# bupt-ai-cz/HIAST

Measured on AMD Instinct MI355X. Metric: self-training images/sec (fwd+bwd+pseudo-label) at 1024x512, higher is better.
Workload: dtype fp16

## Files before the change

hiast_amd/_lib.py:

```python
import ctypes
import os

import torch

_HERE = os.path.dirname(os.path.abspath(__file__))
LIB_PATH = os.environ.get("HIAST_LIB") or os.path.join(_HERE, "csrc", "libhiast_hip.so")

c_int, c_i64, c_f32, c_sz, c_vp = (ctypes.c_int, ctypes.c_int64, ctypes.c_float, ctypes.c_size_t,
                                   ctypes.c_void_p)

SIGNATURES = {
    "hiast_version": (c_int, []),
    "hiast_error_string": (ctypes.c_char_p, [c_int]),
    "hiast_upsample_bilinear_ac_fwd": (c_int, [c_vp, c_vp] + [c_int] * 6 + [c_vp]),
    "hiast_upsample_bilinear_ac_bwd": (c_int, [c_vp, c_vp] + [c_int] * 6 + [c_vp]),
    "hiast_plabel_pass1_workspace_bytes": (c_sz, [c_int]),
    "hiast_plabel_pass1": (c_int, [c_vp] + [c_int] * 6 + [c_vp, c_vp, c_vp, c_vp, c_sz, c_vp]),
    "hiast_plabel_pass2": (c_int, [c_vp, c_vp, c_vp, c_int, c_int, c_i64, c_vp, c_vp, c_vp, c_vp]),
    "hiast_plabel_strided_hist_workspace_bytes": (c_sz, [c_i64, c_int]),
    "hiast_plabel_strided_hist": (c_int, [c_vp, c_vp, c_i64, c_int, c_int, c_vp, c_vp, c_vp, c_vp, c_sz, c_vp]),
    "hiast_tta_fused": (c_int, [c_vp] * 6 + [c_int] * 5 + [c_vp, c_vp, c_vp]),
    "hiast_dinput_fwd": (c_int, [c_vp, c_int, c_vp] + [c_int] * 6 + [c_vp]),
    "hiast_dinput_bwd": (c_int, [c_vp, c_int, c_vp, c_vp, c_vp] + [c_int] * 6 + [c_vp]),
    "hiast_st_loss_workspace_bytes": (c_sz, [c_int] * 6),
# ... 39 lines not shown
    "hiast_conv_wgrad_nhwc": (c_int, [c_vp, c_vp, c_vp] + [c_int] * 9 + [c_vp, c_sz, c_vp]),
    "hiast_conv_wgrad_group_workspace_bytes": (c_sz, [c_vp, c_int]),
    "hiast_conv_wgrad_group_nhwc": (c_int, [c_vp, c_int, c_int, c_vp, c_sz, c_vp]),
    "hiast_conv_wgrad_small_workspace_bytes": (c_sz, [c_int] * 6),
    "hiast_conv_wgrad_small_nhwc": (c_int, [c_vp, c_vp, c_vp] + [c_int] * 9 + [c_vp, c_sz, c_vp]),
    "hiast_pack_conv_weight": (c_int, [c_vp, c_int, c_int, c_int, c_int, c_int, c_vp, c_vp, c_vp]),
    "hiast_bn_nhwc_workspace_bytes": (c_sz, [c_int]),
    "hiast_bn_nhwc_stats": (c_int, [c_vp, c_i64, c_int, c_vp, c_vp, c_sz, c_int, c_vp]),
    "hiast_bn_nhwc_apply": (c_int, [c_vp] * 8 + [ctypes.c_double, c_f32, c_f32, c_int, c_vp, c_vp, c_i64, c_int, c_vp,
                                    c_int, c_vp]),
    "hiast_bn_nhwc_apply_partial": (c_int, [c_vp] * 8 + [c_int, ctypes.c_double, c_f32, c_f32, c_int, c_vp, c_vp, c_i64,
                                            c_int, c_vp, c_int, c_vp]),
    "hiast_bn_nhwc_bwd_stats": (c_int, [c_vp] * 7 + [c_int, c_i64, c_int, c_vp, c_vp, c_sz, c_int, c_vp]),
    "hiast_bn_nhwc_bwd_apply": (c_int, [c_vp] * 8 + [ctypes.c_double, c_int, c_vp, c_vp, c_vp, c_vp, c_i64, c_int, c_int,
                                        c_vp]),
    "hiast_pack_conv_weight_multi": (c_int, [c_vp, c_vp, c_vp, c_int, c_int, c_vp]),
    "hiast_split_planes": (c_int, [c_vp, c_vp, c_i64, c_int, c_int, c_vp]),
    "hiast_stem_tail": (c_int, [c_vp, c_int, c_vp, c_vp, c_vp, c_vp, c_f32, c_vp, c_int, c_int, c_int, c_int, c_int, c_vp]),
    "hiast_stem_eval": (c_int, [c_vp] * 6 + [c_f32, c_vp, c_int, c_int, c_int, c_int, c_vp]),
    "hiast_stem_train_blocks": (c_int, [c_int] * 3),
    "hiast_stem_train_fwd": (c_int, [c_vp, c_vp, c_vp, c_vp, c_int, c_int, c_int, c_int, c_vp]),
    "hiast_stem_wgrad_workspace_bytes": (c_sz, [c_int] * 3),
    "hiast_stem_wgrad": (c_int, [c_vp, c_vp, c_vp, c_int, c_int, c_int, c_int, c_vp, c_sz, c_vp]),
    "hiast_ema_update": (c_int, [c_vp, c_vp, c_vp, c_int, c_f32, c_f32, c_vp]),
    "hiast_normalize_u8": (c_int, [c_vp, c_vp, c_int, c_i64, c_vp, c_vp, c_vp]),
    "hiast_maxpool3x3s2_nhwc_fwd": (c_int, [c_vp, c_vp, c_vp, c_int, c_int, c_int, c_int, c_int, c_vp]),
    "hiast_maxpool3x3s2_nhwc_bwd": (c_int, [c_vp, c_vp, c_vp, c_int, c_int, c_int, c_int, c_int, c_vp]),
    "hiast_multi_copy": (c_int, [c_vp, c_int, c_vp]),
    "hiast_aug_geometry_u8": (c_int, [c_vp] * 6 + [c_int] * 4 + [c_vp]),
    "hiast_aug_hist_u8": (c_int, [c_vp] * 5 + [c_int, c_i64, c_vp]),
# ... 70 lines not shown
```

hiast_amd/csrc/bn_nhwc.hip:

```cpp
#include <hip/hip_bf16.h>

#include "common.h"

namespace hiast {

constexpr int BNH_MAXBLK = 512;
#ifndef BNH_ROWS_PER_BLOCK_PASS
#define BNH_ROWS_PER_BLOCK_PASS 16
#endif
#ifndef BNH_APPLY_MAXBLK
#define BNH_APPLY_MAXBLK 65535
#endif
#ifndef BNH_CONTIG
#define BNH_CONTIG 0
#endif
#if BNH_CONTIG
#define BNH_ROW_WALK(CHUNK)                                                                                              \
    const long long step = (CHUNK);                                                                                      \
    const long long per_blk = ((M + gridDim.x - 1) / gridDim.x + (CHUNK) - 1) / (CHUNK) * (CHUNK);                       \
    const long long lim = (long long)(blockIdx.x + 1) * per_blk < M ? (long long)(blockIdx.x + 1) * per_blk : M;         \
    long long r0 = (long long)blockIdx.x * per_blk + rsub;
#else
#define BNH_ROW_WALK(CHUNK)                                                                                              \
    const long long step = (long long)gridDim.x * (CHUNK);                                                               \
// ... 382 lines not shown
            for (int k = 0; k < 8; ++k) {
                const bool open = GATE == 0 || (GATE == 1 ? yy[k] > 0.f
                                                : (GATE == 3 ? ((bits >> k) & 1u) != 0u : fmaf(xx[k], k0[k], gsh[k]) > 0.f));
                const float gg = open ? g[k] : 0.f;
                g[k] = gg;
                xx[k] = k0[k] * (gg - mg[k] - (xx[k] - mean[k]) * invstd[k] * mgx[k]);
            }
            bnh_store8<F16>(dx + off, xx, nt_out);
            if (DRES) bnh_store8<F16>(dres + off, g, nt_out);
        }
        r0 += step;
        if (r0 < lim) load_rows(r0);
    }
}

static int bnh_nblk(long long M, int C)
{
    const int rpp = 256 / (C / 8);
    long long nb = (M + (long long)rpp * 16 - 1) / ((long long)rpp * 16);
    nb = nb < 1 ? 1 : (nb > BNH_MAXBLK ? BNH_MAXBLK : nb);
    return (int)nb;
}

}

static bool bnh_c_ok(int C) { return C >= 8 && C <= 2048 && (C & (C - 1)) == 0; }

static int bnh_check(const void* x, long long M, int C)
{
    if (!x) return HIAST_E_ARG;
// ... 153 lines not shown
#define L1(G, DRES, F)                                                                                             \
    hipLaunchKernelGGL((hiast::bnh_bwd_apply_kernel<G, DRES, F>), dim3((unsigned)nb), dim3(256), 0, st,             \
                       (const unsigned short*)dy, (const unsigned short*)y, (const unsigned short*)x, gamma, beta,  \
                       save_mean, save_invstd, sums, 1.0 / count, (unsigned short*)dx, (unsigned short*)dres, dgamma, \
                       dbeta, (long long)M, C)
#define L(G, DRES) do { if (f16) L1(G, DRES, true); else L1(G, DRES, false); } while (0)
    if (relu == 1) { if (dres) L(1, true); else L(1, false); }
    else if (relu == 3) { if (dres) L(3, true); else L(3, false); }
    else if (relu == 2) { if (dres) L(2, true); else L(2, false); }
    else { if (dres) L(0, true); else L(0, false); }
#undef L
#undef L1
    HIAST_CHECK_LAUNCH();
    return 0;
}
```

hiast_amd/csrc/misc.hip:

```cpp
#include <hip/hip_bf16.h>

#include <atomic>

#include "common.h"

namespace hiast {

__global__ __launch_bounds__(256) void ema_kernel(const hiast_ema_rec* __restrict__ table,
                                                  const int32_t* __restrict__ chunk_tensor,
                                                  const int64_t* __restrict__ chunk_start,
                                                  float gamma, float omg)
{
    const hiast_ema_rec r = table[chunk_tensor[blockIdx.x]];
    const int64_t s = chunk_start[blockIdx.x];
    const int64_t e = (s + 65536 < r.n) ? s + 65536 : r.n;
    float* __restrict__ d = r.ema;
    const float* __restrict__ p = r.p;
    const bool vec = ((((uintptr_t)d) | ((uintptr_t)p)) & 15) == 0;
    if (vec) {
        const int64_t nv = (e - s) / 4;
        float4* d4 = reinterpret_cast<float4*>(d + s);
        const float4* p4 = reinterpret_cast<const float4*>(p + s);
        for (int64_t i = threadIdx.x; i < nv; i += 256) {
            float4 a = d4[i], b = p4[i];
// ... 348 lines not shown
                for (int k = 0; k < 8; ++k) {
                    const unsigned code = ((k < 4 ? cd.x : cd.y) >> (8 * (k & 3))) & 255u;
                    const float gv = (k & 1) ? H16<F16>::hi(gw[k >> 1]) : H16<F16>::lo(gw[k >> 1]);
                    if (code == pos) acc[k] += gv;
                }
            }
        }
        unsigned pk[4];
#pragma unroll
        for (int q = 0; q < 4; ++q)
            pk[q] = H16<F16>::pack(acc[2 * q], acc[2 * q + 1]);
        *reinterpret_cast<uint4*>(dx + (size_t)pix * C + cg * 8) = make_uint4(pk[0], pk[1], pk[2], pk[3]);
    }
}

}

static int maxpool_cl_check(const void* a, const void* b, const void* c, int B, int H, int W, int C)
{
    if (!a || !b || !c) return HIAST_E_ARG;
    if (B <= 0 || H <= 0 || W <= 0 || C <= 0) return HIAST_E_ARG;
    if (C % 8 != 0 || ((((uintptr_t)a) | ((uintptr_t)b)) & 15) || (((uintptr_t)c) & 7) ||
        (long long)B * H * W * C >= (1ll << 40))
        return HIAST_E_RANGE;
    return 0;
}

extern "C" int hiast_maxpool3x3s2_nhwc_fwd(const void* x, void* y, uint8_t* idx, int B, int H, int W, int C, int fmt,
                                           hiast_stream_t stream)
{
// ... 33 lines not shown
}

extern "C" int hiast_normalize_u8(const uint8_t* img, float* out, int B, int64_t HW, const float* mean, const float* std,
                                  hiast_stream_t stream)
{
    if (!img || !out || !mean || !std) return HIAST_E_ARG;
    if (B <= 0 || HW <= 0) return HIAST_E_ARG;
    if (B > 65535) return HIAST_E_RANGE;
    long long nb = (HW + 256 * 4 - 1) / (256 * 4);
    nb = nb < 1 ? 1 : (nb > 1024 ? 1024 : nb);
    hipLaunchKernelGGL(hiast::normalize_u8_kernel, dim3((unsigned)nb, B), dim3(256), 0, (hipStream_t)stream, img, out,
                       (long long)HW, mean[0], mean[1], mean[2], std[0], std[1], std[2]);
    HIAST_CHECK_LAUNCH();
    return 0;
}
```

hiast_amd/functional.py:

```python
import os

import torch

from . import kernels as K
from . import switches as SW

ASPP_DILATIONS = (6, 12, 18, 24)
H16 = (torch.bfloat16, torch.float16)


class _AsppFn(torch.autograd.Function):

    @staticmethod
    @torch.amp.custom_fwd(device_type="cuda", cast_inputs=torch.float32)
    def forward(ctx, x, w0, w1, w2, w3, b0, b1, b2, b3, dil):
        x = x.contiguous()
        ws = [w.contiguous() for w in (w0, w1, w2, w3)]
        bs = [b.contiguous() for b in (b0, b1, b2, b3)]
        wpack = K.aspp_pack_weights(ws, bs)
        Cout = ws[0].shape[0]
        y = K.aspp_fwd(x, wpack, Cout, dil)
        ctx.save_for_backward(x, wpack)
        ctx.dil = dil
        ctx.cin = x.shape[1]
# ... 299 lines not shown
        else:
            if fused is not None:
                sums = K.bn_nhwc_stats_from_partial(fused)
            else:
                sums = K.bn_nhwc_bwd_stats(dy, y, x, gamma, beta, sm, si, ctx.gate)
            if ctx.world != 1:
                _stat_all_reduce(sums)
        want_p = gamma is not None and (ctx.needs_input_grad[2] or ctx.needs_input_grad[3])
        handoff = ctx.box is not None and ctx.needs_input_grad[1]
        dx, dres, dg, db = K.bn_nhwc_bwd_apply(dy, y, x, gamma, beta, sm, si, sums, ctx.count, ctx.gate,
                                               ctx.has_res and ctx.needs_input_grad[1] and not handoff, want_p)
        if handoff:
            ctx.box["gated"] = (dy, y)
        return (dx, dres, dg if ctx.needs_input_grad[2] else None, db if ctx.needs_input_grad[3] else None,
                None, None, None, None, None, None, None, None, None)


class _ConvNhwcFn(torch.autograd.Function):

    @staticmethod
    @torch.amp.custom_fwd(device_type="cuda")
    def forward(ctx, x, weight, stride, dil, want_stats, box, packed, in_bn=None, wgroup=None, xsum=None, in_bn3=None):
        xv = x.permute(0, 2, 3, 1)
        ctx.in_bn3 = None
        if (in_bn3 is not None and "bn3" in in_bn3 and box is not None and stride == 1 and weight.shape[2] == 1
                and ctx.needs_input_grad[0] and _BN3_FUSION
                and K.xconv_dgrad_gated_bn_stats_ok(x.shape[0] * x.shape[2] * x.shape[3], weight.shape[0], weight.shape[1])):
            ctx.in_bn3 = in_bn3
        ctx.wgroup = wgroup
        ctx.xsum = xsum if (xsum is not None and stride == 1 and ctx.needs_input_grad[0]) else None
# ... 412 lines not shown
            dy = dy.to(ctx.dtype)
        return K.maxpool3x3s2_cl_bwd(dy.contiguous(memory_format=torch.channels_last), idx, *ctx.hw)


def maxpool(x, pool):
    if (x.is_cuda and x.dtype in H16 and _is_cl(x) and x.shape[1] % 8 == 0
            and (pool.kernel_size, pool.stride, pool.padding, pool.dilation, pool.ceil_mode) == (3, 2, 1, 1, False)
            and not pool.return_indices and os.environ.get("HIAST_LIB_MAXPOOL", "0") != "1"):
        return _MaxPool3x3s2ClFn.apply(x)
    return pool(x)


class _SubsampleClFn(torch.autograd.Function):

    @staticmethod
    def forward(ctx, x, s):
        ctx.s, ctx.shape = s, x.shape
        return x[:, :, ::s, ::s].contiguous(memory_format=torch.channels_last)

    @staticmethod
    def backward(ctx, dy):
        g = torch.empty(ctx.shape, dtype=dy.dtype, device=dy.device, memory_format=torch.channels_last).zero_()
        g[:, :, ::ctx.s, ::ctx.s] = dy
        return g, None


def conv_nhwc(x, conv, want_stats=False, box=None, in_bn=None, wgroup=None, xsum=None, in_bn3=None):
    w = conv.weight
    wv = w if wgroup is None else wgroup[2]
    fmt = K.fmt_of(x)
    fwd = conv.__dict__.get("_hiast_packed", {}).get(fmt)
    adj = conv.__dict__.get("_hiast_packed_adj", {}).get(fmt)
    ok = lambda e: e is not None and e[0] == w._version and e[1] == w.data_ptr()
    packed = (fwd[2] if ok(fwd) else None, adj[2] if ok(adj) else None)
    stride = conv.stride[0]
    if conv.kernel_size == (1, 1) and stride != 1:
        x = _SubsampleClFn.apply(x, stride)
        stride = 1
    return _ConvNhwcFn.apply(x, wv, stride, conv.dilation[0], bool(want_stats), box, packed, in_bn,
                             None if wgroup is None else (wgroup[0], wgroup[1]), xsum, in_bn3)


_nbt_batched = [False]


def bn_act(x, bn, res=None, relu=True, partial=None, box=None, stat_box=None):
    training = bn.training or (bn.running_mean is None)
    if training and bn.track_running_stats and bn.num_batches_tracked is not None and not _nbt_batched[0]:
        bn.num_batches_tracked.add_(1)
    momentum = 0.1 if bn.momentum is None else bn.momentum
    if (training and x.dtype in H16 and _is_cl(x) and not x.is_contiguous()
            and K.bn_nhwc_supported(x.shape[1]) and (res is None or (res.dtype == x.dtype and _is_cl(res)))):
        return _BnActNhwcFn.apply(x, res, bn.weight, bn.bias, bn.running_mean, bn.running_var, momentum, bn.eps, relu,
# ... 4 lines not shown
```

hiast_amd/kernels.py:

```python
import ctypes

import numpy as np
import torch

from . import _lib
from . import switches as _SW
from ._lib import NBINS, check


def _stream():
    return ctypes.c_void_p(torch._C._cuda_getCurrentRawStream(torch._C._cuda_getDevice()))


def _ptr(t):
    return ctypes.c_void_p(t.data_ptr()) if t is not None else ctypes.c_void_p(0)


def h2d_async(host, device, out=None):
    stage = torch.from_numpy(np.ascontiguousarray(host)).pin_memory()
    if out is None:
        return stage.to(device, non_blocking=True)
    out.copy_(stage.view(out.dtype).reshape(out.shape) if stage.dtype != out.dtype else stage.reshape(out.shape),
              non_blocking=True)
    return out
# ... 1310 lines not shown
def bn_nhwc_bwd_apply(dy, y, x, gamma, beta, save_mean, save_invstd, sums, count, gate, want_dres, want_dparam):
    xv, M, C = _bnh_view(x, "x")
    dv = _bnh_view(dy, "dy")[0]
    yv = _bnh_view(y, "y")[0] if gate == 1 else (_req(y, torch.uint8, 2, "mask") if gate == 3 else None)
    dx = torch.empty_like(x, memory_format=torch.channels_last)
    dres = torch.empty_like(x, memory_format=torch.channels_last) if want_dres else None
    dg = torch.empty(C, dtype=torch.float32, device=x.device) if want_dparam else None
    db = torch.empty(C, dtype=torch.float32, device=x.device) if want_dparam else None
    check(_lib.load().hiast_bn_nhwc_bwd_apply(_ptr(dv), _ptr(yv), _ptr(xv), _ptr(gamma), _ptr(beta), _ptr(save_mean),
                                              _ptr(save_invstd), _ptr(sums), float(count), int(gate), _ptr(dx),
                                              _ptr(dres), _ptr(dg), _ptr(db), M, C, fmt_of(x), _stream()),
          "hiast_bn_nhwc_bwd_apply")
    return dx, dres, dg, db


_wgrad_ws = {}


def conv_wgrad_supported(Cin, Cout, k, stride):
    return Cin % 256 == 0 and Cout % 256 == 0 and k in (1, 3) and (k == 3 or stride == 1)


def conv_wgrad_preferred(Cin, Cout, k, stride):
    import os
    if not conv_wgrad_supported(Cin, Cout, k, stride):
        return False
    return k == 1 or os.environ.get("HIAST_LIB_WGRAD3", "0") != "1"


def conv_wgrad_small_supported(Cin, Cout, k, stride):
# ... 161 lines not shown
```

hiast_amd/sseg/models/modules/resnet.py:

```python
import os

import torch
import torch.nn as nn
import torch.nn.functional as F

from hiast_amd import functional as HF


def bn_act(bn, x, res=None, relu=True, partial=None):
    if x.is_cuda:
        return HF.bn_act(x, bn, res, relu, partial=partial)
    y = bn(x)
    if res is not None:
        y = y + res
    return F.relu(y) if relu else y


def conv(m, x):
    if x.is_cuda and x.dtype in HF.H16 and HF.conv_nhwc_ok(x, m):
        return HF.conv_nhwc(x, m)
    return m(x)


def conv_bn_act(cv, bn, x, res=None, relu=True, conv_box=None, bn_box=None, in_bn=None, stat_box=None, wgroup=None, xsum=None,
# ... 32 lines not shown
        super().__init__()
        self.conv1 = nn.Conv2d(inplanes, planes, 1, bias=False)
        self.bn1 = nn.BatchNorm2d(planes)
        self.conv2 = nn.Conv2d(planes, planes, 3, stride=stride, padding=dilation, dilation=dilation, bias=False)
        self.bn2 = nn.BatchNorm2d(planes)
        self.conv3 = nn.Conv2d(planes, planes * 4, 1, bias=False)
        self.bn3 = nn.BatchNorm2d(planes * 4)
        self.relu = nn.ReLU(inplace=True)
        self.downsample = downsample

    def forward(self, x):
        xs = None
        if (self.downsample is not None and self.downsample[0].stride == (1, 1) and x.is_cuda and x.dtype in HF.H16
                and self.bn1.training and x.requires_grad and not HF.SW.on("HIAST_NO_XSUM")):
            xs = {}
        idt = x if self.downsample is None else conv_bn_act(self.downsample[0], self.downsample[1], x, relu=False,
                                                            xsum=None if xs is None else (xs, "take"))
        box = {} if (self.downsample is None and not HF.SW.on("HIAST_NO_IDT_HANDOFF")) else None
        sb1, sb2 = {}, {}
        grp, wv = (None, None)
        if x.is_cuda and x.dtype in HF.H16 and self.bn1.training:
            grp, wv = HF.wgroup_weights((self.conv1, self.conv2, self.conv3), x)
        g = (lambda i: (grp, grp["slot"][i], wv[i]) if wv[i] is not None else None) if grp is not None else (lambda i: None)
        o = conv_bn_act(self.conv1, self.bn1, x, conv_box=box, stat_box=sb1, wgroup=g(0),
                        xsum=None if xs is None else (xs, "give"), in_bn3=getattr(x, "_hiast_bn3", None) if box is not None else None)
        o = conv_bn_act(self.conv2, self.bn2, o, in_bn=sb1, stat_box=sb2, wgroup=g(1))
        sb3 = {}
        y = conv_bn_act(self.conv3, self.bn3, o, res=idt, bn_box=box, in_bn=sb2, stat_box=sb3, wgroup=g(2))
        if "bn3" in sb3:
            y._hiast_bn3 = sb3
        return y

    def forward_eval_planes(self, x, fmt):
        from hiast_amd import kernels as K
        PL = 2 if fmt == K.FMT_SPLIT_BF16 else 1
        o = K.igemm_bn_act(x, packed_weight(self.conv1, fmt), PL, self.bn1, None, True)
        if self.downsample is None:
            idt = x
        else:
            dconv, dbn = self.downsample[0], self.downsample[1]
            xs = x if dconv.stride == (1, 1) else x[:, ::dconv.stride[0], ::dconv.stride[1]].contiguous()
            idt = K.igemm_bn_act(xs, packed_weight(dconv, fmt), PL, dbn, None, False)
        o = K.igemm_bn_act(o, packed_weight(self.conv2, fmt), PL, self.bn2, None, True, self.conv2.stride[0],
# ... 160 lines not shown
```

hiast_amd/switches.py:

```python
import os

_NAMES = ("HIAST_NO_BN_MASK", "HIAST_NO_BN_BWD_FUSION", "HIAST_LIB_WGRAD", "HIAST_NO_WGROUP", "HIAST_NO_XSUM",
          "HIAST_NO_IDT_HANDOFF", "HIAST_LIB_STEM")
SWITCHES = {n: os.environ.get(n, "0") == "1" for n in _NAMES}
_OPT_IN_NAMES = ("HIAST_DISC_HIP",)
OPT_IN = {n: os.environ.get(n, "0") == "1" for n in _OPT_IN_NAMES}


def on(name):
    return OPT_IN[name] if name in OPT_IN else SWITCHES[name]
```

include/hiast_hip.h:

```cpp
#ifndef HIAST_HIP_H
#define HIAST_HIP_H

#include <stddef.h>
#include <stdint.h>

#ifdef __cplusplus
extern "C" {
#endif

#define HIAST_ABI_VERSION 6

#define HIAST_E_ARG   (-1)
#define HIAST_E_RANGE (-2)
#define HIAST_E_WS    (-3)

#define HIAST_NBINS 15361
#define HIAST_PROB_FX_SHIFT 30
#define HIAST_MAX_CLASSES 32
#define HIAST_FMT_BF16 1
#define HIAST_FMT_SPLIT_BF16 2
#define HIAST_FMT_FP16 3
#define HIAST_IGNORE 255

typedef void* hiast_stream_t;
// ... 157 lines not shown
int hiast_bn_nhwc_apply_partial(const void* x, const void* res, void* y, const float* gamma, const float* beta,
                                float* running_mean, float* running_var, const float* partial, int nblk, double count,
                                float momentum, float eps, int relu, float* save_mean, float* save_invstd, int64_t M,
                                int C, void* mask, int fmt, hiast_stream_t stream);
int hiast_bn_nhwc_apply(const void* x, const void* res, void* y, const float* gamma, const float* beta,
                        float* running_mean, float* running_var, const double* sums, double count, float momentum,
                        float eps, int relu, float* save_mean, float* save_invstd, int64_t M, int C, void* mask, int fmt,
                        hiast_stream_t stream);
int hiast_bn_nhwc_bwd_stats(const void* dy, const void* y, const void* x, const float* gamma, const float* beta,
                            const float* save_mean, const float* save_invstd, int relu, int64_t M, int C, double* sums,
                            void* workspace, size_t workspace_bytes, int fmt, hiast_stream_t stream);
int hiast_bn_nhwc_bwd_apply(const void* dy, const void* y, const void* x, const float* gamma, const float* beta,
                            const float* save_mean, const float* save_invstd, const double* sums, double count, int relu,
                            void* dx, void* dres, float* dgamma, float* dbeta, int64_t M, int C, int fmt,
                            hiast_stream_t stream);

typedef struct { float* ema; const float* p; int64_t n; } hiast_ema_rec;
int hiast_ema_update(const hiast_ema_rec* table, const int32_t* chunk_tensor,
                     const int64_t* chunk_start, int n_chunks, float gamma,
                     float one_minus_gamma, hiast_stream_t stream);

int hiast_maxpool3x3s2_nhwc_fwd(const void* x, void* y, uint8_t* idx, int B, int H, int W, int C,
                                int fmt , hiast_stream_t stream);
int hiast_maxpool3x3s2_nhwc_bwd(const void* dy, const uint8_t* idx, void* dx, int B, int H, int W, int C, int fmt,
                                hiast_stream_t stream);

int hiast_normalize_u8(const uint8_t* img, float* out, int B, int64_t HW, const float* mean, const float* std,
                       hiast_stream_t stream);

#define HIAST_AUG_REC_WORDS 20
#define HIAST_AUG_MAX_OPS 8
#define HIAST_AUG_OPS_WORDS (4 + 2 * HIAST_AUG_MAX_OPS)
#define HIAST_AUG_OP_LUT 1
#define HIAST_AUG_OP_GRAY 2
#define HIAST_AUG_OP_EQUALIZE 3
int hiast_aug_geometry_u8(const int64_t* recs, const uint8_t* blob, const int32_t* tabs, uint8_t* tmp,
                          uint8_t* img_out, uint8_t* lbl_out, int B, int max_ch, int oh, int ow, hiast_stream_t stream);
int hiast_aug_hist_u8(const int64_t* ops, const uint8_t* blob, const uint8_t* in, uint32_t* hist, uint8_t* eq_lut,
                      int B, int64_t HW, hiast_stream_t stream);
int hiast_aug_colour_u8(const int64_t* ops, const uint8_t* blob, const uint8_t* eq_lut, const uint8_t* in,
// ... 46 lines not shown
```

Before: 143.2.

## Fuse bottleneck downsample BN with conv3 BN into paired apply/backward kernels

Adds paired BatchNorm kernels that apply the conv3 BN and the downsample-branch BN together with the residual add and ReLU in one pass. The backward side computes both BNs' gradient statistics and input gradients from a shared ReLU mask in one pass. The bottleneck block now routes downsampling blocks through this path and extends the x-sum handoff to strided 1x1 downsample convs, adding a strided-add kernel for the backward. The aim is to cut separate elementwise passes over the identity tensor and extra kernel launches. The cost is more code paths, a rounding of the identity branch to fp16 to mirror the unfused version, and a guard-dependent fallback.

```diff
diff --git a/hiast_amd/_lib.py b/hiast_amd/_lib.py
--- a/hiast_amd/_lib.py
+++ b/hiast_amd/_lib.py
@@ -77,6 +77,11 @@
     "hiast_bn_nhwc_bwd_stats": (c_int, [c_vp] * 7 + [c_int, c_i64, c_int, c_vp, c_vp, c_sz, c_int, c_vp]),
     "hiast_bn_nhwc_bwd_apply": (c_int, [c_vp] * 8 + [ctypes.c_double, c_int, c_vp, c_vp, c_vp, c_vp, c_i64, c_int, c_int,
                                         c_vp]),
+    "hiast_bn_nhwc_pair_apply_partial": (c_int, [c_vp] * 9 + [c_int, c_f32, c_f32, c_vp, c_vp] + [c_vp] * 5
+                                         + [c_int, c_f32, c_f32, c_vp, c_vp] + [ctypes.c_double, c_i64, c_int, c_int, c_vp]),
+    "hiast_bn_nhwc_pair_bwd_stats": (c_int, [c_vp] * 8 + [c_i64, c_int, c_vp, c_vp, c_vp, c_sz, c_int, c_vp]),
+    "hiast_bn_nhwc_pair_bwd_apply": (c_int, [c_vp] * 12 + [ctypes.c_double] + [c_vp] * 6 + [c_i64, c_int, c_int, c_vp]),
+    "hiast_strided_add_nhwc": (c_int, [c_vp, c_vp, c_int, c_int, c_int, c_int, c_int, c_int, c_vp]),
     "hiast_pack_conv_weight_multi": (c_int, [c_vp, c_vp, c_vp, c_int, c_int, c_vp]),
     "hiast_split_planes": (c_int, [c_vp, c_vp, c_i64, c_int, c_int, c_vp]),
     "hiast_stem_tail": (c_int, [c_vp, c_int, c_vp, c_vp, c_vp, c_vp, c_f32, c_vp, c_int, c_int, c_int, c_int, c_int, c_vp]),
diff --git a/hiast_amd/csrc/bn_nhwc.hip b/hiast_amd/csrc/bn_nhwc.hip
--- a/hiast_amd/csrc/bn_nhwc.hip
+++ b/hiast_amd/csrc/bn_nhwc.hip
@@ -420,6 +420,264 @@
     }
 }
 
+
+template <bool F16>
+__device__ __forceinline__ float bnh_r16(float v)
+{
+    asm volatile("" : "+v"(v));
+    return H16<F16>::dec(H16<F16>::enc(v));
+}
+
+template <bool F16>
+__global__ __launch_bounds__(256) void bnh_pair_apply_kernel(
+    const unsigned short* __restrict__ x3, const unsigned short* __restrict__ xd, unsigned short* __restrict__ y,
+    unsigned char* __restrict__ mask, const float* __restrict__ gamma3, const float* __restrict__ beta3,
+    const float* __restrict__ mean3, const float* __restrict__ invstd3, const float* __restrict__ gammad,
+    const float* __restrict__ betad, const float* __restrict__ meand, const float* __restrict__ invstdd, long long M, int C)
+{
+    const int G = C >> 3, RPP = 256 / G;
+    const bool nt_out = (long long)M * C * 2 >= H_NT_MIN_BYTES;
+    const int cg = threadIdx.x % G, rsub = threadIdx.x / G;
+    constexpr int UNR = BNH_UNR_APPLY;
+    const long long stride = RPP;
+    BNH_ROW_WALK(RPP * UNR)
+
+    uint4 r3[UNR], rd[UNR];
+    auto load_rows = [&](long long rb) {
+#pragma unroll
+        for (int u = 0; u < UNR; ++u) {
+            const long long r = rb + u * stride;
+            const size_t off = (size_t)(r < lim ? r : (rb < lim ? rb : 0)) * C + cg * 8;
+            r3[u] = bnh_ld16<1>(x3 + off);
+            rd[u] = bnh_ld16<1>(xd + off);
+        }
+    };
+    load_rows(r0);
+    float sc3[8], sh3[8], scd[8], shd[8];
+    {
+        float gm[8], bt[8], mn[8], is[8];
+        bnh_param8(gamma3, mean3, cg * 8, 1.0f, gm);
+        bnh_param8(beta3, mean3, cg * 8, 0.0f, bt);
+        bnh_param8(mean3, mean3, cg * 8, 0.f, mn);
+        bnh_param8(invstd3, mean3, cg * 8, 0.f, is);
+#pragma unroll
+        for (int k = 0; k < 8; ++k) {
+            sc3[k] = gm[k] * is[k];
+            sh3[k] = fmaf(-mn[k], sc3[k], bt[k]);
+        }
+        bnh_param8(gammad, meand, cg * 8, 1.0f, gm);
+        bnh_param8(betad, meand, cg * 8, 0.0f, bt);
+        bnh_param8(meand, meand, cg * 8, 0.f, mn);
+        bnh_param8(invstdd, meand, cg * 8, 0.f, is);
+#pragma unroll
+        for (int k = 0; k < 8; ++k) {
+            scd[k] = gm[k] * is[k];
+            shd[k] = fmaf(-mn[k], scd[k], bt[k]);
+        }
+    }
+    while (r0 < lim) {
+#pragma unroll
+        for (int u = 0; u < UNR; ++u) {
+            const long long r = r0 + u * stride;
+            if (r >= lim) break;
+            const size_t off = (size_t)r * C + cg * 8;
+            float v[8], d[8];
+            bnh_unpack8<F16>(r3[u], v);
+            bnh_unpack8<F16>(rd[u], d);
+            unsigned bits = 0;
+#pragma unroll
+            for (int k = 0; k < 8; ++k) {
+                const float idt = bnh_r16<F16>(fmaf(d[k], scd[k], shd[k]));
+                float o = fmaf(v[k], sc3[k], sh3[k]);
+                o += idt;
+                o = o > 0.f ? o : 0.f;
+                bits |= (o > 0.f ? 1u : 0u) << k;
+                v[k] = o;
+            }
+            bnh_store8<F16>(y + off, v, nt_out);
+            mask[(size_t)r * G + cg] = (unsigned char)bits;
+        }
+        r0 += step;
+        if (r0 < lim) load_rows(r0);
+    }
+}
+
+template <bool BOTH, bool F16>
+__global__ __launch_bounds__(256) void bnh_pair_partial_kernel(
+    const unsigned short* __restrict__ g, const unsigned char* __restrict__ mask, const unsigned short* __restrict__ x3,
+    const unsigned short* __restrict__ xd, const float* __restrict__ mean3, const float* __restrict__ invstd3,
+    const float* __restrict__ meand, const float* __restrict__ invstdd, long long M, int C,
+    float* __restrict__ partial3, float* __restrict__ partiald)
+{
+    constexpr int NS = BOTH ? 3 : 2;
+    __shared__ float s_red[256 * 8 * NS];
+    const int G = C >> 3, RPP = 256 / G;
+    const int cg = threadIdx.x % G, rsub = threadIdx.x / G;
+    float s1[8], s23[8], s2d[8], m3[8], i3[8], md[8], id[8];
+#pragma unroll
+    for (int k = 0; k < 8; ++k) { s1[k] = 0.f; s23[k] = 0.f; s2d[k] = 0.f; m3[k] = 0.f; i3[k] = 0.f; }
+    constexpr int UNR = BNH_UNR_PART;
+    const long long stride = RPP;
+    BNH_ROW_WALK(RPP * UNR)
+
+    uint4 rg[UNR], r3[UNR], rd[UNR];
+    unsigned rbits[UNR];
+    auto load_rows = [&](long long rb) {
+#pragma unroll
+        for (int u = 0; u < UNR; ++u) {
+            const long long r = rb + u * stride;
+            const long long rc = r < lim ? r : (rb < lim ? rb : 0);
+            const size_t off = (size_t)rc * C + cg * 8;
+            rg[u] = bnh_ld16<0>(g + off);
+            rbits[u] = mask[(size_t)rc * G + cg];
+            if (BOTH) r3[u] = bnh_ld16<0>(x3 + off);
+            rd[u] = bnh_ld16<0>(xd + off);
+        }
+    };
+    load_rows(r0);
+    if (BOTH) {
+        bnh_param8(mean3, mean3, cg * 8, 0.f, m3);
+        bnh_param8(invstd3, mean3, cg * 8, 0.f, i3);
+    }
+    bnh_param8(meand, meand, cg * 8, 0.f, md);
+    bnh_param8(invstdd, meand, cg * 8, 0.f, id);
+    while (r0 < lim) {
+#pragma unroll
+        for (int u = 0; u < UNR; ++u) {
+            if (r0 + u * stride >= lim) break;
+            float v[8], a[8], b[8];
+            bnh_unpack8<F16>(rg[u], v);
+            const unsigned bits = rbits[u];
+            if (BOTH) bnh_unpack8<F16>(r3[u], a);
+            bnh_unpack8<F16>(rd[u], b);
+#pragma unroll
+            for (int k = 0; k < 8; ++k) {
+                const float gg = ((bits >> k) & 1u) != 0u ? v[k] : 0.f;
+                s1[k] += gg;
+                if (BOTH) s23[k] = fmaf(gg, (a[k] - m3[k]) * i3[k], s23[k]);
+                s2d[k] = fmaf(gg, (b[k] - md[k]) * id[k], s2d[k]);
+            }
+        }
+        r0 += step;
+        if (r0 < lim) load_rows(r0);
+    }
+#pragma unroll
+    for (int k = 0; k < 8; ++k) {
+        s_red[threadIdx.x * 8 * NS + k] = s1[k];
+        s_red[threadIdx.x * 8 * NS + 8 + k] = s2d[k];
+        if (BOTH) s_red[threadIdx.x * 8 * NS + 16 + k] = s23[k];
+    }
+    __syncthreads();
+    if (rsub == 0) {
+        const size_t o = ((size_t)blockIdx.x * C + cg * 8) * 2;
+#pragma unroll
+        for (int k = 0; k < 8; ++k) {
+            float t1 = 0.f, t2 = 0.f, t3 = 0.f;
+            for (int j = 0; j < RPP; ++j) {
+                t1 += s_red[(j * G + cg) * 8 * NS + k];
+                t2 += s_red[(j * G + cg) * 8 * NS + 8 + k];
+                if (BOTH) t3 += s_red[(j * G + cg) * 8 * NS + 16 + k];
+            }
+            partiald[o + 2 * k] = t1;
+            partiald[o + 2 * k + 1] = t2;
+            if (BOTH) {
+                partial3[o + 2 * k] = t1;
+                partial3[o + 2 * k + 1] = t3;
+            }
+        }
+    }
+}
+
+template <bool F16>
+__global__ __launch_bounds__(256) void bnh_pair_bwd_apply_kernel(
+    const unsigned short* __restrict__ g, const unsigned char* __restrict__ mask, const unsigned short* __restrict__ x3,
+    const unsigned short* __restrict__ xd, const float* __restrict__ gamma3, const float* __restrict__ mean3,
+    const float* __restrict__ invstd3, const double* __restrict__ sums3, const float* __restrict__ gammad,
+    const float* __restrict__ meand, const float* __restrict__ invstdd, const double* __restrict__ sumsd, double inv_count,
+    unsigned short* __restrict__ dx3, unsigned short* __restrict__ dxd, float* __restrict__ dgamma3,
+    float* __restrict__ dbeta3, float* __restrict__ dgammad, float* __restrict__ dbetad, long long M, int C)
+{
+    const int G = C >> 3, RPP = 256 / G;
+    const bool nt_out = (long long)M * C * 2 >= H_NT_MIN_BYTES;
+    const int cg = threadIdx.x % G, rsub = threadIdx.x / G;
+    constexpr int UNR = 2;
+    const long long stride = RPP;
+    BNH_ROW_WALK(RPP * UNR)
+
+    uint4 rg[UNR], r3[UNR], rd[UNR];
+    unsigned rbits[UNR];
+    auto load_rows = [&](long long rb) {
+#pragma unroll
+        for (int u = 0; u < UNR; ++u) {
+            const long long r = rb + u * stride;
+            const long long rc = r < lim ? r : (rb < lim ? rb : 0);
+            const size_t off = (size_t)rc * C + cg * 8;
+            rg[u] = bnh_ld16<2>(g + off);
+            rbits[u] = mask[(size_t)rc * G + cg];
+            r3[u] = bnh_ld16<2>(x3 + off);
+            rd[u] = bnh_ld16<2>(xd + off);
+        }
+    };
+    load_rows(r0);
+    float m3[8], i3[8], k3[8], mg3[8], mgx3[8], md[8], id[8], kd[8], mgd[8], mgxd[8];
+    {
+        float gm[8];
+        bnh_param8(mean3, mean3, cg * 8, 0.f, m3);
+        bnh_param8(invstd3, mean3, cg * 8, 0.f, i3);
+        bnh_param8(gamma3, mean3, cg * 8, 1.0f, gm);
+        const double2* sp = reinterpret_cast<const double2*>(sums3) + cg * 8;
+#pragma unroll
+        for (int k = 0; k < 8; ++k) {
+            const double2 ss = sp[k];
+            if (blockIdx.x == 0 && rsub == 0) {
+                if (dbeta3) dbeta3[cg * 8 + k] = (float)ss.x;
+                if (dgamma3) dgamma3[cg * 8 + k] = (float)ss.y;
+            }
+            k3[k] = gm[k] * i3[k];
+            mg3[k] = (float)(ss.x * inv_count);
+            mgx3[k] = (float)(ss.y * inv_count);
+        }
+        bnh_param8(meand, meand, cg * 8, 0.f, md);
+        bnh_param8(invstdd, meand, cg * 8, 0.f, id);
+        bnh_param8(gammad, meand, cg * 8, 1.0f, gm);
+        sp = reinterpret_cast<const double2*>(sumsd) + cg * 8;
+#pragma unroll
+        for (int k = 0; k < 8; ++k) {
+            const double2 ss = sp[k];
+            if (blockIdx.x == 0 && rsub == 0) {
+                if (dbetad) dbetad[cg * 8 + k] = (float)ss.x;
+                if (dgammad) dgammad[cg * 8 + k] = (float)ss.y;
+            }
+            kd[k] = gm[k] * id[k];
+            mgd[k] = (float)(ss.x * inv_count);
+            mgxd[k] = (float)(ss.y * inv_count);
+        }
+    }
+    while (r0 < lim) {
+#pragma unroll
+        for (int u = 0; u < UNR; ++u) {
+            const long long r = r0 + u * stride;
+            if (r >= lim) break;
+            const size_t off = (size_t)r * C + cg * 8;
+            float gg[8], a[8], b[8];
+            bnh_unpack8<F16>(rg[u], gg);
+            const unsigned bits = rbits[u];
+            bnh_unpack8<F16>(r3[u], a);
+            bnh_unpack8<F16>(rd[u], b);
+#pragma unroll
+            for (int k = 0; k < 8; ++k) {
+                const float gk = ((bits >> k) & 1u) != 0u ? gg[k] : 0.f;
+                a[k] = k3[k] * (gk - mg3[k] - (a[k] - m3[k]) * i3[k] * mgx3[k]);
+                b[k] = kd[k] * (gk - mgd[k] - (b[k] - md[k]) * id[k] * mgxd[k]);
+            }
+            bnh_store8<F16>(dx3 + off, a, nt_out);
+            bnh_store8<F16>(dxd + off, b, nt_out);
+        }
+        r0 += step;
+        if (r0 < lim) load_rows(r0);
+    }
+}
+
 static int bnh_nblk(long long M, int C)
 {
     const int rpp = 256 / (C / 8);
@@ -603,3 +861,105 @@
     HIAST_CHECK_LAUNCH();
     return 0;
 }
+
+
+static long long bnh_apply_nb(long long M, int C)
+{
+    const int rpp = 256 / (C / 8);
+    long long nb = (M + (long long)rpp * BNH_ROWS_PER_BLOCK_PASS - 1) / ((long long)rpp * BNH_ROWS_PER_BLOCK_PASS);
+    return nb < 1 ? 1 : (nb > BNH_APPLY_MAXBLK ? BNH_APPLY_MAXBLK : nb);
+}
+
+extern "C" int hiast_bn_nhwc_pair_apply_partial(
+    const void* x3, const void* xd, void* y, void* mask, const float* gamma3, const float* beta3, float* running_mean3,
+    float* running_var3, const float* partial3, int nblk3, float momentum3, float eps3, float* save_mean3, float* save_invstd3,
+    const float* gammad, const float* betad, float* running_meand, float* running_vard, const float* partiald, int nblkd,
+    float momentumd, float epsd, float* save_meand, float* save_invstdd, double count, int64_t M, int C, int fmt,
+    hiast_stream_t stream)
+{
+    BNH_FMT_CHECK();
+    int e = bnh_check(x3, M, C);
+    if (e) return e;
+    if (!xd || !y || !mask || !partial3 || !partiald || !save_mean3 || !save_invstd3 || !save_meand || !save_invstdd ||
+        count <= 0 || nblk3 <= 0 || nblkd <= 0)
+        return HIAST_E_ARG;
+    if ((((uintptr_t)y) | ((uintptr_t)xd)) & 15) return HIAST_E_RANGE;
+    hipStream_t st = (hipStream_t)stream;
+    hipLaunchKernelGGL(hiast::bnh_finalize_prep_kernel, dim3(C / 2), dim3(256), 0, st, partiald, nblkd, C, count, momentumd,
+                       epsd, running_meand, running_vard, save_meand, save_invstdd);
+    HIAST_CHECK_LAUNCH();
+    hipLaunchKernelGGL(hiast::bnh_finalize_prep_kernel, dim3(C / 2), dim3(256), 0, st, partial3, nblk3, C, count, momentum3,
+                       eps3, running_mean3, running_var3, save_mean3, save_invstd3);
+    HIAST_CHECK_LAUNCH();
+    const unsigned nb = (unsigned)bnh_apply_nb(M, C);
+#define L(F)                                                                                                            \
+    hipLaunchKernelGGL((hiast::bnh_pair_apply_kernel<F>), dim3(nb), dim3(256), 0, st, (const unsigned short*)x3,         \
+                       (const unsigned short*)xd, (unsigned short*)y, (unsigned char*)mask, gamma3, beta3,               \
+                       (const float*)save_mean3, (const float*)save_invstd3, gammad, betad, (const float*)save_meand,    \
+                       (const float*)save_invstdd, (long long)M, C)
+    if (f16) L(true); else L(false);
+#undef L
+    HIAST_CHECK_LAUNCH();
+    return 0;
+}
+
+extern "C" int hiast_bn_nhwc_pair_bwd_stats(const void* dy, const void* mask, const void* x3, const void* xd,
+                                            const float* save_mean3, const float* save_invstd3, const float* save_meand,
+                                            const float* save_invstdd, int64_t M, int C, double* sums3, double* sumsd,
+                                            void* workspace, size_t workspace_bytes, int fmt, hiast_stream_t stream)
+{
+    BNH_FMT_CHECK();
+    int e = bnh_check(xd, M, C);
+    if (e) return e;
+    if (!dy || !mask || !save_meand || !save_invstdd || !sumsd || !workspace) return HIAST_E_ARG;
+    if (x3 && (!save_mean3 || !save_invstd3 || !sums3)) return HIAST_E_ARG;
+    if ((((uintptr_t)dy) | ((uintptr_t)x3)) & 15) return HIAST_E_RANGE;
+    const int nblk = hiast::bnh_nblk(M, C);
+    const size_t one = (size_t)nblk * C * 2 * sizeof(float);
+    if (workspace_bytes < (x3 ? 2 : 1) * one) return HIAST_E_WS;
+    float* pd = (float*)workspace;
+    float* p3 = pd + (size_t)nblk * C * 2;
+    hipStream_t st = (hipStream_t)stream;
+#define L(BOTH, F)                                                                                                      \
+    hipLaunchKernelGGL((hiast::bnh_pair_partial_kernel<BOTH, F>), dim3(nblk), dim3(256), 0, st, (const unsigned short*)dy, \
+                       (const unsigned char*)mask, (const unsigned short*)x3, (const unsigned short*)xd, save_mean3,     \
+                       save_invstd3, save_meand, save_invstdd, (long long)M, C, p3, pd)
+    if (x3) { if (f16) L(true, true); else L(true, false); }
+    else { if (f16) L(false, true); else L(false, false); }
+#undef L
+    HIAST_CHECK_LAUNCH();
+    if (x3) {
+        hipLaunchKernelGGL(hiast::bnh_finalize_kernel, dim3(C * 2 / 16), dim3(256), 0, st, (const float*)p3, nblk, C, sums3);
+        HIAST_CHECK_LAUNCH();
+    }
+    hipLaunchKernelGGL(hiast::bnh_finalize_kernel, dim3(C * 2 / 16), dim3(256), 0, st, (const float*)pd, nblk, C, sumsd);
+    HIAST_CHECK_LAUNCH();
+    return 0;
+}
+
+extern "C" int hiast_bn_nhwc_pair_bwd_apply(const void* dy, const void* mask, const void* x3, const void* xd,
+                                            const float* gamma3, const float* save_mean3, const float* save_invstd3,
+                                            const double* sums3, const float* gammad, const float* save_meand,
+                                            const float* save_invstdd, const double* sumsd, double count, void* dx3, void* dxd,
+                                            float* dgamma3, float* dbeta3, float* dgammad, float* dbetad, int64_t M, int C,
+                                            int fmt, hiast_stream_t stream)
+{
+    BNH_FMT_CHECK();
+    int e = bnh_check(x3, M, C);
+    if (e) return e;
+    if (!dy || !mask || !xd || !save_mean3 || !save_invstd3 || !sums3 || !save_meand || !save_invstdd || !sumsd || !dx3 ||
+        !dxd || count <= 0)
+        return HIAST_E_ARG;
+    if ((((uintptr_t)dy) | ((uintptr_t)xd) | ((uintptr_t)dx3) | ((uintptr_t)dxd)) & 15) return HIAST_E_RANGE;
+    const unsigned nb = (unsigned)bnh_apply_nb(M, C);
+    hipStream_t st = (hipStream_t)stream;
+#define L(F)                                                                                                            \
+    hipLaunchKernelGGL((hiast::bnh_pair_bwd_apply_kernel<F>), dim3(nb), dim3(256), 0, st, (const unsigned short*)dy,     \
+                       (const unsigned char*)mask, (const unsigned short*)x3, (const unsigned short*)xd, gamma3,         \
+                       save_mean3, save_invstd3, sums3, gammad, save_meand, save_invstdd, sumsd, 1.0 / count,            \
+                       (unsigned short*)dx3, (unsigned short*)dxd, dgamma3, dbeta3, dgammad, dbetad, (long long)M, C)
+    if (f16) L(true); else L(false);
+#undef L
+    HIAST_CHECK_LAUNCH();
+    return 0;
+}
diff --git a/hiast_amd/csrc/misc.hip b/hiast_amd/csrc/misc.hip
--- a/hiast_amd/csrc/misc.hip
+++ b/hiast_amd/csrc/misc.hip
@@ -386,6 +386,29 @@
     }
 }
 
+template <bool F16>
+__global__ __launch_bounds__(256) void strided_add_cl_kernel(unsigned short* __restrict__ dx,
+                                                             const unsigned short* __restrict__ dy, int B, int H, int W, int C,
+                                                             int s, int Hs, int Ws)
+{
+    const int G = C >> 3;
+    const long long total = (long long)B * Hs * Ws * G;
+    for (long long i = (long long)blockIdx.x * 256 + threadIdx.x; i < total; i += (long long)gridDim.x * 256) {
+        const int cg = (int)(i % G);
+        const long long pix = i / G;
+        const int xo = (int)(pix % Ws), yo = (int)((pix / Ws) % Hs), b = (int)(pix / ((long long)Ws * Hs));
+        unsigned short* p = dx + ((((size_t)b * H + (size_t)yo * s) * W + (size_t)xo * s) * C + cg * 8);
+        const uint4 a = *reinterpret_cast<const uint4*>(p);
+        const uint4 g = *reinterpret_cast<const uint4*>(dy + (size_t)pix * C + cg * 8);
+        const unsigned aw[4] = {a.x, a.y, a.z, a.w}, gw[4] = {g.x, g.y, g.z, g.w};
+        unsigned pk[4];
+#pragma unroll
+        for (int q = 0; q < 4; ++q)
+            pk[q] = H16<F16>::pack(H16<F16>::lo(aw[q]) + H16<F16>::lo(gw[q]), H16<F16>::hi(aw[q]) + H16<F16>::hi(gw[q]));
+        *reinterpret_cast<uint4*>(p) = make_uint4(pk[0], pk[1], pk[2], pk[3]);
+    }
+}
+
 }
 
 static int maxpool_cl_check(const void* a, const void* b, const void* c, int B, int H, int W, int C)
@@ -449,3 +472,24 @@
     HIAST_CHECK_LAUNCH();
     return 0;
 }
+
+extern "C" int hiast_strided_add_nhwc(void* dx, const void* dy, int B, int H, int W, int C, int s, int fmt,
+                                      hiast_stream_t stream)
+{
+    if (fmt != HIAST_FMT_BF16 && fmt != HIAST_FMT_FP16) return HIAST_E_RANGE;
+    if (!dx || !dy) return HIAST_E_ARG;
+    if (B <= 0 || H <= 0 || W <= 0 || C <= 0 || s <= 0) return HIAST_E_ARG;
+    if (C % 8 != 0 || ((((uintptr_t)dx) | ((uintptr_t)dy)) & 15) || (long long)B * H * W * C >= (1ll << 40))
+        return HIAST_E_RANGE;
+    const int Hs = (H - 1) / s + 1, Ws = (W - 1) / s + 1;
+    long long nb = ((long long)B * Hs * Ws * (C / 8) + 255) / 256;
+    nb = nb > 16384 ? 16384 : nb;
+    if (fmt == HIAST_FMT_FP16)
+        hipLaunchKernelGGL(hiast::strided_add_cl_kernel<true>, dim3((unsigned)nb), dim3(256), 0, (hipStream_t)stream,
+                           (unsigned short*)dx, (const unsigned short*)dy, B, H, W, C, s, Hs, Ws);
+    else
+        hipLaunchKernelGGL(hiast::strided_add_cl_kernel<false>, dim3((unsigned)nb), dim3(256), 0, (hipStream_t)stream,
+                           (unsigned short*)dx, (const unsigned short*)dy, B, H, W, C, s, Hs, Ws);
+    HIAST_CHECK_LAUNCH();
+    return 0;
+}
diff --git a/hiast_amd/functional.py b/hiast_amd/functional.py
--- a/hiast_amd/functional.py
+++ b/hiast_amd/functional.py
@@ -337,6 +337,67 @@
             ctx.box["gated"] = (dy, y)
         return (dx, dres, dg if ctx.needs_input_grad[2] else None, db if ctx.needs_input_grad[3] else None,
                 None, None, None, None, None, None, None, None, None)
+
+
+class _BnPairNhwcFn(torch.autograd.Function):
+
+    @staticmethod
+    def forward(ctx, y3, yd, gamma3, beta3, gammad, betad, partial3, partiald, bn3, bnd, stat_box):
+        count = float(y3.shape[0] * y3.shape[2] * y3.shape[3])
+        mom = lambda bn: 0.1 if bn.momentum is None else bn.momentum
+        out, mask, st3, std = K.bn_nhwc_pair_apply_partial(
+            y3, yd, (gamma3, beta3, bn3.running_mean, bn3.running_var, mom(bn3), bn3.eps),
+            (gammad, betad, bnd.running_mean, bnd.running_var, mom(bnd), bnd.eps), partial3, partiald, count)
+        ctx.save_for_backward(y3, yd, mask, gamma3, gammad, st3[0], st3[1], std[0], std[1])
+        ctx.count = count
+        ctx.stat_box = None
+        if stat_box is not None:
+            left = stat_box.pop("bwd_sums", None)
+            if left is not None:
+                _stat_wait(left[1])
+            stat_box.pop("bwd_partial", None)
+            stat_box["bn3"] = (y3.detach(), mask, st3[0], st3[1])
+            stat_box["world"] = 1
+            ctx.stat_box = stat_box
+        return out
+
+    @staticmethod
+    def backward(ctx, dy):
+        y3, yd, mask, gamma3, gammad, sm3, si3, smd, sid = ctx.saved_tensors
+        if dy.dtype != y3.dtype:
+            dy = dy.to(y3.dtype)
+        dy = dy.contiguous(memory_format=torch.channels_last)
+        fused = ctx.stat_box.pop("bwd_partial", None) if ctx.stat_box is not None else None
+        if fused is not None:
+            sums3 = K.bn_nhwc_stats_from_partial(fused)
+            _, sumsd = K.bn_nhwc_pair_bwd_stats(dy, mask, None, yd, None, (smd, sid))
+        else:
+            sums3, sumsd = K.bn_nhwc_pair_bwd_stats(dy, mask, y3, yd, (sm3, si3), (smd, sid))
+        need = ctx.needs_input_grad
+        want3 = gamma3 is not None and (need[2] or need[3])
+        wantd = gammad is not None and (need[4] or need[5])
+        dx3, dxd, (dg3, db3), (dgd, dbd) = K.bn_nhwc_pair_bwd_apply(dy, mask, y3, yd, gamma3, (sm3, si3), sums3, gammad,
+                                                                    (smd, sid), sumsd, ctx.count, want3, wantd)
+        return (dx3 if need[0] else None, dxd if need[1] else None, dg3 if need[2] else None, db3 if need[3] else None,
+                dgd if need[4] else None, dbd if need[5] else None, None, None, None, None, None)
+
+
+def boundary_fusion():
+    return not SW.on("HIAST_NO_BOUNDARY_FUSION")
+
+
+def bn_pair_ok(y3, yd, bn3, bnd):
+    return (boundary_fusion() and not SW.on("HIAST_NO_BN_MASK") and bn3.training and bnd.training
+            and y3.is_cuda and y3.dtype in H16 and yd.dtype == y3.dtype and yd.shape == y3.shape
+            and _is_cl(y3) and not y3.is_contiguous() and _is_cl(yd) and not yd.is_contiguous()
+            and K.bn_nhwc_supported(y3.shape[1]) and _sync_world(bn3) == 1 and _sync_world(bnd) == 1)
+
+
+def bn_pair(y3, bn3, partial3, yd, bnd, partiald, stat_box=None):
+    for bn in (bn3, bnd):
+        if bn.track_running_stats and bn.num_batches_tracked is not None and not _nbt_batched[0]:
+            bn.num_batches_tracked.add_(1)
+    return _BnPairNhwcFn.apply(y3, yd, bn3.weight, bn3.bias, bnd.weight, bnd.bias, partial3, partiald, bn3, bnd, stat_box)
 
 
 class _ConvNhwcFn(torch.autograd.Function):
@@ -779,15 +840,26 @@
 class _SubsampleClFn(torch.autograd.Function):
 
     @staticmethod
-    def forward(ctx, x, s):
+    def forward(ctx, x, s, xsum=None):
         ctx.s, ctx.shape = s, x.shape
+        ctx.xsum = xsum if (xsum is not None and ctx.needs_input_grad[0] and x.dtype in H16 and _is_cl(x)) else None
+        if ctx.xsum is not None:
+            ctx.xsum["taker"] = True
         return x[:, :, ::s, ::s].contiguous(memory_format=torch.channels_last)
 
     @staticmethod
     def backward(ctx, dy):
+        other = None
+        if ctx.xsum is not None:
+            other = ctx.xsum.pop("dx", None)
+            ctx.xsum["taken"] = True
+        if other is not None and other.shape == ctx.shape and other.dtype == dy.dtype and _is_cl(other):
+            return K.strided_add_cl_(other, dy.contiguous(memory_format=torch.channels_last), ctx.s), None, None
         g = torch.empty(ctx.shape, dtype=dy.dtype, device=dy.device, memory_format=torch.channels_last).zero_()
         g[:, :, ::ctx.s, ::ctx.s] = dy
-        return g, None
+        if other is not None:
+            g = g + other
+        return g, None, None
 
 
 def conv_nhwc(x, conv, want_stats=False, box=None, in_bn=None, wgroup=None, xsum=None, in_bn3=None):
@@ -800,8 +872,8 @@
     packed = (fwd[2] if ok(fwd) else None, adj[2] if ok(adj) else None)
     stride = conv.stride[0]
     if conv.kernel_size == (1, 1) and stride != 1:
-        x = _SubsampleClFn.apply(x, stride)
-        stride = 1
+        x = _SubsampleClFn.apply(x, stride, xsum[0] if (xsum is not None and xsum[1] == "take") else None)
+        stride, xsum = 1, None
     return _ConvNhwcFn.apply(x, wv, stride, conv.dilation[0], bool(want_stats), box, packed, in_bn,
                              None if wgroup is None else (wgroup[0], wgroup[1]), xsum, in_bn3)
 
diff --git a/hiast_amd/kernels.py b/hiast_amd/kernels.py
--- a/hiast_amd/kernels.py
+++ b/hiast_amd/kernels.py
@@ -1348,6 +1348,77 @@
     return dx, dres, dg, db
 
 
+def bn_nhwc_pair_apply_partial(x3, xd, bn3, bnd, partial3, partiald, count):
+    v3, M, C = _bnh_view(x3, "x3")
+    vd, M2, C2 = _bnh_view(xd, "xd")
+    assert (M2, C2) == (M, C) and xd.dtype == x3.dtype
+    for p in (partial3, partiald):
+        _req(p, torch.float32, 3, "partial")
+        assert p.shape[1] == C and p.shape[2] == 2
+    y = torch.empty_like(x3, memory_format=torch.channels_last)
+    mask = torch.empty((M, C // 8), dtype=torch.uint8, device=x3.device)
+    st = [torch.empty(C, dtype=torch.float32, device=x3.device) for _ in range(4)]
+    g3, b3, rm3, rv3, mo3, ep3 = bn3
+    gd, bd, rmd, rvd, mod, epd = bnd
+    check(_lib.load().hiast_bn_nhwc_pair_apply_partial(
+        _ptr(v3), _ptr(vd), _ptr(y), _ptr(mask), _ptr(g3), _ptr(b3), _ptr(rm3), _ptr(rv3), _ptr(partial3), partial3.shape[0],
+        float(mo3), float(ep3), _ptr(st[0]), _ptr(st[1]), _ptr(gd), _ptr(bd), _ptr(rmd), _ptr(rvd), _ptr(partiald),
+        partiald.shape[0], float(mod), float(epd), _ptr(st[2]), _ptr(st[3]), float(count), M, C, fmt_of(x3), _stream()),
+        "hiast_bn_nhwc_pair_apply_partial")
+    return y, mask, (st[0], st[1]), (st[2], st[3])
+
+
+def bn_nhwc_pair_bwd_stats(dy, mask, x3, xd, stat3, statd):
+    vd, M, C = _bnh_view(xd, "xd")
+    dv, M2, C2 = _bnh_view(dy, "dy")
+    assert (M2, C2) == (M, C)
+    _req(mask, torch.uint8, 2, "mask")
+    assert tuple(mask.shape) == (M, C // 8)
+    v3 = None
+    if x3 is not None:
+        v3, M3, C3 = _bnh_view(x3, "x3")
+        assert (M3, C3) == (M, C)
+    sums3 = torch.empty((C, 2), dtype=torch.float64, device=xd.device) if x3 is not None else None
+    sumsd = torch.empty((C, 2), dtype=torch.float64, device=xd.device)
+    key = (C, xd.device, "pair")
+    ws = _bnh_ws.get(key)
+    if ws is None:
+        ws = _bnh_ws[key] = torch.empty(2 * (_lib.load().hiast_bn_nhwc_workspace_bytes(C) // 4), dtype=torch.float32,
+                                         device=xd.device)
+    sm3, si3 = stat3 if x3 is not None else (None, None)
+    check(_lib.load().hiast_bn_nhwc_pair_bwd_stats(_ptr(dv), _ptr(mask), _ptr(v3), _ptr(vd), _ptr(sm3), _ptr(si3),
+                                                   _ptr(statd[0]), _ptr(statd[1]), M, C, _ptr(sums3), _ptr(sumsd), _ptr(ws),
+                                                   ws.numel() * 4, fmt_of(xd), _stream()), "hiast_bn_nhwc_pair_bwd_stats")
+    return sums3, sumsd
+
+
+def bn_nhwc_pair_bwd_apply(dy, mask, x3, xd, gamma3, stat3, sums3, gammad, statd, sumsd, count, want_p3, want_pd):
+    v3, M, C = _bnh_view(x3, "x3")
+    vd = _bnh_view(xd, "xd")[0]
+    dv = _bnh_view(dy, "dy")[0]
+    _req(mask, torch.uint8, 2, "mask")
+    assert tuple(mask.shape) == (M, C // 8) and vd.shape == v3.shape == dv.shape
+    dx3 = torch.empty_like(x3, memory_format=torch.channels_last)
+    dxd = torch.empty_like(xd, memory_format=torch.channels_last)
+    new = lambda want: torch.empty(C, dtype=torch.float32, device=x3.device) if want else None
+    dg3, db3, dgd, dbd = new(want_p3), new(want_p3), new(want_pd), new(want_pd)
+    check(_lib.load().hiast_bn_nhwc_pair_bwd_apply(
+        _ptr(dv), _ptr(mask), _ptr(v3), _ptr(vd), _ptr(gamma3), _ptr(stat3[0]), _ptr(stat3[1]), _ptr(sums3), _ptr(gammad),
+        _ptr(statd[0]), _ptr(statd[1]), _ptr(sumsd), float(count), _ptr(dx3), _ptr(dxd), _ptr(dg3), _ptr(db3), _ptr(dgd),
+        _ptr(dbd), M, C, fmt_of(x3), _stream()), "hiast_bn_nhwc_pair_bwd_apply")
+    return dx3, dxd, (dg3, db3), (dgd, dbd)
+
+
+def strided_add_cl_(dx, dy, s):
+    xv, _, C = _bnh_view(dx, "dx")
+    yv = _bnh_view(dy, "dy")[0]
+    B, H, W, _ = xv.shape
+    assert dy.dtype == dx.dtype and tuple(yv.shape) == (B, (H - 1) // s + 1, (W - 1) // s + 1, C)
+    check(_lib.load().hiast_strided_add_nhwc(_ptr(xv), _ptr(yv), B, H, W, C, int(s), fmt_of(dx), _stream()),
+          "hiast_strided_add_nhwc")
+    return dx
+
+
 _wgrad_ws = {}
 
 
diff --git a/hiast_amd/sseg/models/modules/resnet.py b/hiast_amd/sseg/models/modules/resnet.py
--- a/hiast_amd/sseg/models/modules/resnet.py
+++ b/hiast_amd/sseg/models/modules/resnet.py
@@ -70,8 +70,21 @@
         if (self.downsample is not None and self.downsample[0].stride == (1, 1) and x.is_cuda and x.dtype in HF.H16
                 and self.bn1.training and x.requires_grad and not HF.SW.on("HIAST_NO_XSUM")):
             xs = {}
-        idt = x if self.downsample is None else conv_bn_act(self.downsample[0], self.downsample[1], x, relu=False,
-                                                            xsum=None if xs is None else (xs, "take"))
+        elif (self.downsample is not None and self.downsample[0].stride != (1, 1) and self.downsample[0].kernel_size == (1, 1)
+                and x.is_cuda and x.dtype in HF.H16 and self.bn1.training and self.downsample[1].training and x.requires_grad
+                and HF._sync_world(self.bn1) == 1 and HF.boundary_fusion() and not HF.SW.on("HIAST_NO_XSUM")
+                and HF.conv_nhwc_ok(x, self.downsample[0]) and HF.conv_nhwc_ok(x, self.conv1)):
+            xs = {}
+        dpair = None
+        if (self.downsample is not None and HF.boundary_fusion() and x.is_cuda and x.dtype in HF.H16
+                and self.downsample[1].training and self.bn3.training and HF.conv_nhwc_ok(x, self.downsample[0])
+                and HF._sync_world(self.bn3) == 1 and HF._sync_world(self.downsample[1]) == 1
+                and not HF.SW.on("HIAST_NO_BN_MASK")):
+            dpair = HF.conv_nhwc(x, self.downsample[0], want_stats=True, xsum=None if xs is None else (xs, "take"))
+            idt = None
+        else:
+            idt = x if self.downsample is None else conv_bn_act(self.downsample[0], self.downsample[1], x, relu=False,
+                                                                xsum=None if xs is None else (xs, "take"))
         box = {} if (self.downsample is None and not HF.SW.on("HIAST_NO_IDT_HANDOFF")) else None
         sb1, sb2 = {}, {}
         grp, wv = (None, None)
@@ -82,7 +95,17 @@
                         xsum=None if xs is None else (xs, "give"), in_bn3=getattr(x, "_hiast_bn3", None) if box is not None else None)
         o = conv_bn_act(self.conv2, self.bn2, o, in_bn=sb1, stat_box=sb2, wgroup=g(1))
         sb3 = {}
-        y = conv_bn_act(self.conv3, self.bn3, o, res=idt, bn_box=box, in_bn=sb2, stat_box=sb3, wgroup=g(2))
+        if dpair is not None and HF.conv_nhwc_ok(o, self.conv3):
+            y3, p3 = HF.conv_nhwc(o, self.conv3, want_stats=True, in_bn=sb2, wgroup=g(2))
+            if HF.bn_pair_ok(y3, dpair[0], self.bn3, self.downsample[1]):
+                y = HF.bn_pair(y3, self.bn3, p3, dpair[0], self.downsample[1], dpair[1], stat_box=sb3)
+            else:
+                idt = HF.bn_act(dpair[0], self.downsample[1], None, False, partial=dpair[1])
+                y = HF.bn_act(y3, self.bn3, idt, True, partial=p3, box=box, stat_box=sb3)
+        else:
+            if dpair is not None:
+                idt = HF.bn_act(dpair[0], self.downsample[1], None, False, partial=dpair[1])
+            y = conv_bn_act(self.conv3, self.bn3, o, res=idt, bn_box=box, in_bn=sb2, stat_box=sb3, wgroup=g(2))
         if "bn3" in sb3:
             y._hiast_bn3 = sb3
         return y
diff --git a/hiast_amd/switches.py b/hiast_amd/switches.py
--- a/hiast_amd/switches.py
+++ b/hiast_amd/switches.py
@@ -5,7 +5,12 @@
 SWITCHES = {n: os.environ.get(n, "0") == "1" for n in _NAMES}
 _OPT_IN_NAMES = ("HIAST_DISC_HIP",)
 OPT_IN = {n: os.environ.get(n, "0") == "1" for n in _OPT_IN_NAMES}
+_MORE_NAMES = ("HIAST_NO_BOUNDARY_FUSION",)
+MORE = {n: os.environ.get(n, "0") == "1" for n in _MORE_NAMES}
 
 
 def on(name):
-    return OPT_IN[name] if name in OPT_IN else SWITCHES[name]
+    for d in (OPT_IN, MORE):
+        if name in d:
+            return d[name]
+    return SWITCHES[name]
diff --git a/include/hiast_hip.h b/include/hiast_hip.h
--- a/include/hiast_hip.h
+++ b/include/hiast_hip.h
@@ -195,6 +195,21 @@
                             const float* save_mean, const float* save_invstd, const double* sums, double count, int relu,
                             void* dx, void* dres, float* dgamma, float* dbeta, int64_t M, int C, int fmt,
                             hiast_stream_t stream);
+int hiast_bn_nhwc_pair_apply_partial(const void* x3, const void* xd, void* y, void* mask, const float* gamma3,
+                                     const float* beta3, float* running_mean3, float* running_var3, const float* partial3,
+                                     int nblk3, float momentum3, float eps3, float* save_mean3, float* save_invstd3,
+                                     const float* gammad, const float* betad, float* running_meand, float* running_vard,
+                                     const float* partiald, int nblkd, float momentumd, float epsd, float* save_meand,
+                                     float* save_invstdd, double count, int64_t M, int C, int fmt, hiast_stream_t stream);
+int hiast_bn_nhwc_pair_bwd_stats(const void* dy, const void* mask, const void* x3, const void* xd, const float* save_mean3,
+                                 const float* save_invstd3, const float* save_meand, const float* save_invstdd, int64_t M,
+                                 int C, double* sums3, double* sumsd, void* workspace, size_t workspace_bytes, int fmt,
+                                 hiast_stream_t stream);
+int hiast_bn_nhwc_pair_bwd_apply(const void* dy, const void* mask, const void* x3, const void* xd, const float* gamma3,
+                                 const float* save_mean3, const float* save_invstd3, const double* sums3, const float* gammad,
+                                 const float* save_meand, const float* save_invstdd, const double* sumsd, double count,
+                                 void* dx3, void* dxd, float* dgamma3, float* dbeta3, float* dgammad, float* dbetad, int64_t M,
+                                 int C, int fmt, hiast_stream_t stream);
 
 typedef struct { float* ema; const float* p; int64_t n; } hiast_ema_rec;
 int hiast_ema_update(const hiast_ema_rec* table, const int32_t* chunk_tensor,
@@ -205,6 +220,7 @@
                                 int fmt , hiast_stream_t stream);
 int hiast_maxpool3x3s2_nhwc_bwd(const void* dy, const uint8_t* idx, void* dx, int B, int H, int W, int C, int fmt,
                                 hiast_stream_t stream);
+int hiast_strided_add_nhwc(void* dx, const void* dy, int B, int H, int W, int C, int s, int fmt, hiast_stream_t stream);
 
 int hiast_normalize_u8(const uint8_t* img, float* out, int B, int64_t HW, const float* mean, const float* std,
                        hiast_stream_t stream);
```

Result: no change. 144.1, median of 3 (+0.7%).
